# KikeM/romtime

Hardware: AMD Instinct MI355X
Metric: snapshot-DoF/s for POD build (higher is better)
Workload: dtype f64

## Files before the change

### include/romtime_hip.h

```cpp
#ifndef ROMTIME_HIP_H
#define ROMTIME_HIP_H

#include <stdint.h>

#ifdef __cplusplus
extern "C" {
#endif

typedef struct rt_ctx rt_ctx;

#define RT_OK 0
#define RT_ERR_ARG (-1)
#define RT_ERR_HIP (-2)
#define RT_ERR_UNSUPPORTED (-3)
#define RT_WARN_ZERO_NORM 1
#define RT_WARN_SINGULAR 2

#define RT_ROW_MAJOR 0
#define RT_COL_MAJOR 1

int rt_version(void);
int rt_ctx_create(rt_ctx** out, int device);
void rt_ctx_destroy(rt_ctx* ctx);
int rt_ctx_set_stream(rt_ctx* ctx, void* hip_stream);
int rt_ctx_synchronize(rt_ctx* ctx);
const char* rt_last_error(rt_ctx* ctx);
int rt_last_launch_info(rt_ctx* ctx, int64_t* info3);

int rt_ctx_set_profile(rt_ctx* ctx, int on);
int rt_ctx_set_option(rt_ctx* ctx, const char* name, int value);

int rt_stream_create_cu_range(int device, int first_cu_per_xcd, int n_cu_per_xcd, void** stream);
int rt_stream_destroy(void* stream);
int rt_last_gemm_ms(rt_ctx* ctx, double* ms);
int rt_ctx_get_counter(rt_ctx* ctx, const char* name, int64_t* value);
int rt_last_gram_ms(rt_ctx* ctx, double* ms);
int rt_gram_plan_info(int num_cus, int64_t n_rows, int64_t n_cols, int* out);


int rt_gram(rt_ctx* ctx, const double* X, int64_t n_rows, int64_t n_cols, int64_t ld, int layout,
            double* G);

int rt_gram_scale(rt_ctx* ctx, double* G, int64_t n, double* colnorm, int normalize, int* status_flag);

int rt_pod_orth(rt_ctx* ctx, const double* X, int64_t n_rows, int64_t n_cols, int64_t ld, int layout, int64_t num,
                double tol, int normalize, double* Q, int64_t q_cols, int64_t* r_out, double* s_host,
                double* energy_host, int* levels_out);

int rt_pod_enqueue(rt_ctx* ctx, const double* X, int64_t n_rows, int64_t n_cols, int64_t ld, int layout, int64_t k,
                   int normalize, double* G, double* colnorm, double* lam, int* status2, double* Z, double* Zs, double* Q);

int rt_pod_backproject_weights(rt_ctx* ctx, const double* Z, int64_t n, int64_t k, const double* colnorm, const double* lam,
                               double* Zs);

int rt_gemm_tn(rt_ctx* ctx, const double* A, int64_t lda, int a_layout, const double* B, int64_t ldb,
               int b_layout, int64_t N, int64_t m, int64_t n, double* C, int64_t ldc);

int rt_gemm_nn(rt_ctx* ctx, const double* X, int64_t ldx, int x_layout, const double* T, int64_t ldt,
               int64_t N, int64_t n, int64_t k, double* Y, int64_t ldy, int y_layout);
int rt_gemm_nn_axpby(rt_ctx* ctx, const double* X, int64_t ldx, int x_layout, const double* T, int64_t ldt,
                     int64_t N, int64_t n, int64_t k, double alpha, double beta, double* Y, int64_t ldy,
                     int y_layout);

int rt_rank_update(rt_ctx* ctx, const double* Ysrc, int64_t ldys, const double* colscale, const double* X, int64_t ldx,
                   const double* T, int64_t ldt, int64_t N, int64_t k, int64_t n, double alpha, double* Ydst,
                   int64_t ldyd);

int rt_transpose(rt_ctx* ctx, const double* src, int64_t rows, int64_t cols, int64_t ld_src, double* dst,
                 int64_t ld_dst);


int rt_deim_greedy(rt_ctx* ctx, const double* Phi, int64_t N, int64_t m, int64_t ld, int layout,
                   int64_t* idx, double* PT_U, double* margin);


int rt_csr_spmm(rt_ctx* ctx, const int64_t* indptr, const int64_t* indices, const double* data, int64_t N,
                const double* V, int64_t ldv, int64_t r, double* Y, int64_t ldy);

int rt_project_csr(rt_ctx* ctx, const int64_t* indptr, const int64_t* indices, const double* data, int64_t N,
                   const double* V, int64_t ldv, int64_t r, double* AN);

int rt_project_csr_batched(rt_ctx* ctx, const int64_t* indptr, const int64_t* indices,
                           const double* data_batch, int64_t ld_data, int data_layout, int64_t B, int64_t N,
                           const double* V, int64_t ldv, int64_t r, double* AN_batch);

int rt_project_stage_info(rt_ctx* ctx, const int64_t* indptr, const int64_t* indices, int64_t N, int64_t* records,
                          int* any_unwindowed);


int rt_dense_solve_batched(rt_ctx* ctx, double* K, double* rhs, int64_t r, int64_t B, int* info);
int rt_dense_solve_multi(rt_ctx* ctx, const double* K, int64_t r, const double* B, double* X, int64_t nrhs, int* info);


int rt_tracked_solve_batched(rt_ctx* ctx, const double* K, double* Xinv, double* rhs, int64_t r, int64_t B, int have_prev,
                             int* info);

#define RT_SOLVER_DIRECT 0
#define RT_SOLVER_GMRES 1
typedef struct {
  double rtol, atol;
  int64_t restart, maxiter;
} rt_gmres_opts;
int rt_gmres_batched(rt_ctx* ctx, const double* K, const double* b, double* x, int64_t r, int64_t B,
                     const rt_gmres_opts* opts, int64_t* info, int* iters);
int rt_ctx_set_reduced_solver(rt_ctx* ctx, int kind, const rt_gmres_opts* opts);

typedef struct {
  int64_t N, nnz, r, n_mu, nt;
  double dt;
  int bdf2;
  const int64_t* indptr;
  const int64_t* indices;
  const double* V;
  const double* mass_values;
  int64_t n_terms;
  const double* term_values;
  const double* term_coef;
  const double* tril_values;
  int64_t n_rhs;
  const double* rhs_terms;
// ... 97 lines not shown
```

### romtime_amd/_lib.py

```python
from __future__ import annotations

import ctypes as C
import os
import threading
import weakref

_HERE = os.path.dirname(os.path.abspath(__file__))
LIB_PATH = os.path.join(_HERE, "lib", "libromtime_hip.so")

ROW_MAJOR, COL_MAJOR = 0, 1
RT_OK = 0
WARN_ZERO_NORM, WARN_SINGULAR = 1, 2
EIG_BLOCKED_OK, EIG_BLOCKED_NOT_REDUCIBLE, EIG_BLOCKED_SOLVE_FAILED = 0, 1, 2

_p = C.c_void_p
_i64 = C.c_int64
_int = C.c_int

SOLVER_DIRECT, SOLVER_GMRES = 0, 1


class GmresOpts(C.Structure):

    _fields_ = [("rtol", C.c_double), ("atol", C.c_double), ("restart", _i64), ("maxiter", _i64)]


SIGNATURES = {
    "rt_version": (_int, []),
    "rt_ctx_create": (_int, [C.POINTER(_p), _int]),
    "rt_ctx_destroy": (None, [_p]),
    "rt_ctx_set_stream": (_int, [_p, _p]),
    "rt_ctx_synchronize": (_int, [_p]),
    "rt_last_error": (C.c_char_p, [_p]),
    "rt_last_launch_info": (_int, [_p, C.POINTER(_i64)]),
    "rt_ctx_set_profile": (_int, [_p, _int]),
    "rt_ctx_set_option": (_int, [_p, C.c_char_p, _int]),
    "rt_last_gemm_ms": (_int, [_p, C.POINTER(C.c_double)]),
    "rt_last_gram_ms": (_int, [_p, C.POINTER(C.c_double)]),
    "rt_gram_plan_info": (_int, [_int, _i64, _i64, C.POINTER(_int)]),
    "rt_ctx_get_counter": (_int, [_p, C.c_char_p, C.POINTER(_i64)]),
    "rt_stream_create_cu_range": (_int, [_int, _int, _int, C.POINTER(_p)]),
    "rt_stream_destroy": (_int, [_p]),
    "rt_last_sweep_stats": (_int, [_p, C.POINTER(_i64)]),
    "rt_gram": (_int, [_p, _p, _i64, _i64, _i64, _int, _p]),
    "rt_gram_scale": (_int, [_p, _p, _i64, _p, _int, _p]),
    "rt_pod_backproject_weights": (_int, [_p, _p, _i64, _i64, _p, _p, _p]),
    "rt_pod_enqueue": (_int, [_p, _p, _i64, _i64, _i64, _int, _i64, _int, _p, _p, _p, _p, _p, _p, _p]),
    "rt_pod_orth": (_int, [_p, _p, _i64, _i64, _i64, _int, _i64, C.c_double, _int, _p, _i64, C.POINTER(_i64), _p, _p,
                           C.POINTER(_int)]),
    "rt_gemm_tn": (_int, [_p, _p, _i64, _int, _p, _i64, _int, _i64, _i64, _i64, _p, _i64]),
    "rt_gemm_nn": (_int, [_p, _p, _i64, _int, _p, _i64, _i64, _i64, _i64, _p, _i64, _int]),
    "rt_rank_update": (_int, [_p, _p, _i64, _p, _p, _i64, _p, _i64, _i64, _i64, _i64, C.c_double, _p, _i64]),
    "rt_gemm_nn_axpby": (_int, [_p, _p, _i64, _int, _p, _i64, _i64, _i64, _i64, C.c_double, C.c_double, _p, _i64, _int]),
    "rt_transpose": (_int, [_p, _p, _i64, _i64, _i64, _p, _i64]),
    "rt_deim_greedy": (_int, [_p, _p, _i64, _i64, _i64, _int, _p, _p, _p]),
    "rt_csr_spmm": (_int, [_p, _p, _p, _p, _i64, _p, _i64, _i64, _p, _i64]),
    "rt_project_csr": (_int, [_p, _p, _p, _p, _i64, _p, _i64, _i64, _p]),
    "rt_project_csr_batched": (_int, [_p, _p, _p, _p, _i64, _int, _i64, _i64, _p, _i64, _i64, _p]),
    "rt_project_stage_info": (_int, [_p, _p, _p, _i64, C.POINTER(_i64), C.POINTER(_int)]),
    "rt_dense_solve_batched": (_int, [_p, _p, _p, _i64, _i64, _p]),
    "rt_dense_solve_multi": (_int, [_p, _p, _i64, _p, _p, _i64, _p]),
    "rt_tracked_solve_batched": (_int, [_p, _p, _p, _p, _i64, _i64, _int, _p]),
    "rt_gmres_batched": (_int, [_p, _p, _p, _p, _i64, _i64, C.POINTER(GmresOpts), _p, _p]),
    "rt_ctx_set_reduced_solver": (_int, [_p, _int, C.POINTER(GmresOpts)]),
    "rt_rom_bdf_sweep": (_int, [_p, _p, _p]),
    "rt_hrom_bdf_sweep": (_int, [_p, _p, _p]),
    "rt_trajectory_errors": (_int, [_p, _p, _i64, _p, _i64, _i64, _p, _i64, _int, _i64, _i64, _i64, _i64, _i64, _p, _p]),
    "rt_trajectory_integrals": (_int, [_p, _p, _i64, _p, _p, _i64, _i64, _p, _i64, _i64, _i64, _i64, _int, C.POINTER(C.c_double), _p]),
    "rt_trajectory_integrals_plan_info": (_int, [_int, _p, _i64, _p, _p, _i64, _i64, _p, _i64, _i64, _i64, _i64, _int,
                                                 C.POINTER(C.c_double), _p, C.POINTER(_i64)]),
    "rt_interpolation_errors": (_int, [_p, _p, _i64, C.POINTER(_i64), _i64, _p, _i64, _int, _i64, _i64, _i64, _i64, C.c_double, _p, _p]),
    "rt_interpolation_errors_plan_info": (_int, [_int, _p, _i64, C.POINTER(_i64), _i64, _p, _i64, _int, _i64, _i64, _i64, _i64,
                                                 C.c_double, _p, _p, C.POINTER(_i64)]),
    "rt_p1_local_assembly": (_int, [_p, _int, _i64, _p, _p, _i64, _i64, _p, _p, _int, _p, _p]),
    "rt_p1_fom_bdf_sweep": (_int, [_p, _p, _p, _i64, _i64, _p]),
    "rt_p1_fom_bdf_sweep_plan_info": (_int, [_int, _p, _i64, _i64, C.POINTER(_i64)]),
    "rt_p1_fom_bdf_sweep_certified": (_int, [_p, _p, _p, _i64, _i64, C.c_double, _p, _p]),
    "rt_p1_fom_bdf_sweep_certified_plan_info": (_int, [_int, _p, _i64, _i64, C.POINTER(_i64)]),
    "rt_trajectory_residuals": (_int, [_p, _p, _p, _i64, _i64, _p, _i64, _i64, _p, _p, _p]),
    "rt_trajectory_residuals_plan_info": (_int, [_int, _p, _p, _i64, _i64, _p, _i64, _i64, _p, _p, _p, C.POINTER(_i64)]),
    "rt_sym_eig_values": (_int, [_p, _p, _i64, _p, _p]),
    "rt_sym_eig_values_part": (_int, [_p, _p, _i64, _i64, _i64, _p, _p]),
    "rt_sym_eig_vectors": (_int, [_p, _i64, _i64, _p, _p]),
    "rt_sym_eig_blocked_plan_info": (_int, [_i64, _i64, C.POINTER(_i64), C.POINTER(_i64)]),
    "rt_sym_eig_blocked": (_int, [_p, _p, _i64, C.c_double, _i64, _p, _p, C.POINTER(_i64), C.POINTER(_i64), C.POINTER(_int)]),
    "rt_sym_jacobi_eigh": (_int, [_p, _p, _i64, _p, _p, _int, C.POINTER(_int), _p]),
    "rt_host_jacobi_eigh": (_int, [_p, _i64, _p, _p, _int, C.POINTER(_int)]),
    "rt_bench_mfma_f64": (_int, [_p, _int, C.POINTER(C.c_double)]),
    "rt_bench_copy": (_int, [_p, _p, _p, _i64, _int, C.POINTER(C.c_double)]),
}



class SweepDesc(C.Structure):

    _fields_ = [("N", _i64), ("nnz", _i64), ("r", _i64), ("n_mu", _i64), ("nt", _i64), ("dt", C.c_double),
                ("bdf2", _int), ("indptr", _p), ("indices", _p), ("V", _p), ("mass_values", _p), ("n_terms", _i64),
                ("term_values", _p), ("term_coef", _p), ("tril_values", _p), ("n_rhs", _i64), ("rhs_terms", _p),
                ("rhs_coef", _p)]


class HSweepDesc(C.Structure):

    _fields_ = [("r", _i64), ("n_mu", _i64), ("nt", _i64), ("dt", C.c_double), ("bdf2", _int), ("m_mass", _i64),
                ("m_lin", _i64), ("m_nl", _i64), ("m_rhs", _i64), ("Z", _p), ("Zf", _p), ("F_mass", _p), ("F_lin", _p),
                ("F_rhs", _p), ("W", _p), ("C_nl", _p), ("S_nl", _p)]


class FomDesc(C.Structure):

    _fields_ = [("nx", _i64), ("n_mu", _i64), ("nt", _i64), ("first_step", _i64), ("dt", C.c_double), ("bdf2", _int),
                ("state_in_w", _int), ("tab", _p), ("u_init", _p)]


_lib = None
_lock = threading.Lock()


class RomtimeHipError(RuntimeError):
    pass


# ... 157 lines not shown
```

### romtime_amd/csrc/api.hip

```cpp
#include "common.h"

#include <chrono>
#include <new>

namespace {

int grow(rt_ctx* ctx, void** buf, size_t* have, size_t bytes, void** out) {
  if (bytes > *have) {
    RT_HIP_CHECK(ctx, hipStreamSynchronize(ctx->stream));
    if (*buf) RT_HIP_CHECK(ctx, hipFree(*buf));
    *buf = nullptr;
    *have = 0;
    const size_t want = (bytes + ((size_t)1 << 20) - 1) & ~(((size_t)1 << 20) - 1);
    RT_HIP_CHECK(ctx, hipMalloc(buf, want));
    *have = want;
  }
  *out = *buf;
  return RT_OK;
}

__global__ void gram_scale_kernel(double* __restrict__ G, int n, double* __restrict__ colnorm, int normalize,
                                  int* status_flag) {
  const long idx = (long)blockIdx.x * blockDim.x + threadIdx.x;
  if (idx >= (long)n * n) return;
// ... 73 lines not shown
      for (int it = 0; it < iters; ++it) {
#pragma unroll
        for (int rep = 0; rep < 2; ++rep)
#pragma unroll
          for (int i = 0; i < 8; ++i) a[i] = fma(a[i], m, c);
      }
#pragma unroll
      for (int i = 0; i < 8; ++i) s += a[i];
    }
    if (mode & 4) {
      unsigned a[8];
#pragma unroll
      for (int i = 0; i < 8; ++i) a[i] = threadIdx.x * 2654435761u + i;
      for (int it = 0; it < iters; ++it) {
#pragma unroll
        for (int rep = 0; rep < 2; ++rep)
#pragma unroll
          for (int i = 0; i < 8; ++i) a[i] = (a[i] ^ (a[i] >> 3)) + 0x9e3779b9u;
      }
#pragma unroll
      for (int i = 0; i < 8; ++i) s += (double)a[i];
    }
    if (mode & 8) {
      int idx = threadIdx.x & 63;
      double a = 0.0;
      for (int it = 0; it < iters; ++it) {
#pragma unroll
        for (int i = 0; i < 16; ++i) a += lds[(idx + 64 * i) & 2047];
        idx = (idx + 1) & 63;
      }
      s += a;
    }
  }
  if (s == -1.2345) sink[0] = s;
}

__global__ __launch_bounds__(256) void copy_kernel(double4* __restrict__ dst, const double4* __restrict__ src, long n4) {
  const long stride = (long)gridDim.x * blockDim.x;
  for (long i = (long)blockIdx.x * blockDim.x + threadIdx.x; i < n4; i += stride) dst[i] = src[i];
}

}

int rt_scratch(rt_ctx* ctx, size_t bytes, void** out) { return grow(ctx, &ctx->scratch, &ctx->scratch_bytes, bytes, out); }
int rt_scratch2(rt_ctx* ctx, size_t bytes, void** out) {
  ++ctx->scratch2_gen;
  return grow(ctx, &ctx->scratch2, &ctx->scratch2_bytes, bytes, out);
}

int rt_func_lds(rt_ctx* ctx, const void* fn, int bytes) {
  for (const void* f : ctx->lds_done)
    if (f == fn) return RT_OK;
  RT_HIP_CHECK(ctx, hipFuncSetAttribute(fn, hipFuncAttributeMaxDynamicSharedMemorySize, bytes));
  ctx->lds_done.push_back(fn);
  return RT_OK;
}

int rt_profile_begin(rt_ctx* ctx, bool also_gram) {
  if (!ctx->profile) return RT_OK;
  if (!ctx->ev0) {
    RT_HIP_CHECK(ctx, hipEventCreate(&ctx->ev0));
    RT_HIP_CHECK(ctx, hipEventCreate(&ctx->ev1));
  }
  if (also_gram && !ctx->gev0) {
    RT_HIP_CHECK(ctx, hipEventCreate(&ctx->gev0));
    RT_HIP_CHECK(ctx, hipEventCreate(&ctx->gev1));
  }
  RT_HIP_CHECK(ctx, hipEventRecord(ctx->ev0, ctx->stream));
  if (also_gram) RT_HIP_CHECK(ctx, hipEventRecord(ctx->gev0, ctx->stream));
  return RT_OK;
}

int rt_profile_end(rt_ctx* ctx, bool also_gram) {
  if (!ctx->profile) return RT_OK;
  RT_HIP_CHECK(ctx, hipEventRecord(ctx->ev1, ctx->stream));
  if (also_gram) RT_HIP_CHECK(ctx, hipEventRecord(ctx->gev1, ctx->stream));
  ctx->ev_valid = true;
  if (also_gram) ctx->gev_valid = true;
  return RT_OK;
}

extern "C" {

int rt_version(void) { return 420; }

int rt_ctx_create(rt_ctx** out, int device) {
  if (!out) return RT_ERR_ARG;
  *out = nullptr;
  int count = 0;
  if (hipGetDeviceCount(&count) != hipSuccess || device < 0 || device >= count) return RT_ERR_HIP;
  if (hipSetDevice(device) != hipSuccess) return RT_ERR_HIP;
  rt_ctx* ctx = new (std::nothrow) rt_ctx();
  if (!ctx) return RT_ERR_HIP;
  ctx->device = device;
  hipDeviceProp_t prop;
  if (hipGetDeviceProperties(&prop, device) == hipSuccess) ctx->num_cus = ctx->device_cus = prop.multiProcessorCount;
  if (hipMalloc(reinterpret_cast<void**>(&ctx->dev_counters), sizeof(long) * RT_N_COUNTERS) != hipSuccess ||
      hipMemset(ctx->dev_counters, 0, sizeof(long) * RT_N_COUNTERS) != hipSuccess) {
    delete ctx;
    return RT_ERR_HIP;
  }
  *out = ctx;
  return RT_OK;
}

void rt_ctx_destroy(rt_ctx* ctx) {
  if (!ctx) return;
  (void)hipSetDevice(ctx->device);
  (void)hipDeviceSynchronize();
  if (ctx->scratch) (void)hipFree(ctx->scratch);
  if (ctx->scratch2) (void)hipFree(ctx->scratch2);
  if (ctx->dev_counters) (void)hipFree(ctx->dev_counters);
  if (ctx->gram_pace) (void)hipFree(ctx->gram_pace);
  if (ctx->ev0) (void)hipEventDestroy(ctx->ev0);
  if (ctx->ev1) (void)hipEventDestroy(ctx->ev1);
  if (ctx->gev0) (void)hipEventDestroy(ctx->gev0);
  if (ctx->gev1) (void)hipEventDestroy(ctx->gev1);
  delete ctx;
}

int rt_ctx_set_stream(rt_ctx* ctx, void* hip_stream) {
  if (!ctx) return RT_ERR_ARG;
  ctx->stream = static_cast<hipStream_t>(hip_stream);
  return RT_OK;
}

int rt_stream_create_cu_range(int device, int first_cu_per_xcd, int n_cu_per_xcd, void** stream) {
  if (!stream) return RT_ERR_ARG;
  *stream = nullptr;
  hipDeviceProp_t prop;
  if (hipSetDevice(device) != hipSuccess || hipGetDeviceProperties(&prop, device) != hipSuccess) return RT_ERR_HIP;
  const int per_xcd = prop.multiProcessorCount / 8;
  if (first_cu_per_xcd < 0 || n_cu_per_xcd < 1 || first_cu_per_xcd + n_cu_per_xcd > per_xcd) return RT_ERR_ARG;
  const int words = (prop.multiProcessorCount + 31) / 32;
  std::vector<uint32_t> mask((size_t)words, 0u);
  for (int cu = first_cu_per_xcd; cu < first_cu_per_xcd + n_cu_per_xcd; ++cu)
    for (int xcd = 0; xcd < 8; ++xcd) {
      const int bit = cu * 8 + xcd;
      mask[bit >> 5] |= 1u << (bit & 31);
    }
  hipStream_t st = nullptr;
  if (hipExtStreamCreateWithCUMask(&st, (uint32_t)words, mask.data()) != hipSuccess) return RT_ERR_HIP;
  *stream = st;
  return RT_OK;
}

int rt_stream_destroy(void* stream) {
  if (!stream) return RT_ERR_ARG;
  return hipStreamDestroy(static_cast<hipStream_t>(stream)) == hipSuccess ? RT_OK : RT_ERR_HIP;
}

int rt_ctx_synchronize(rt_ctx* ctx) {
  if (!ctx) return RT_ERR_ARG;
  RT_HIP_CHECK(ctx, hipStreamSynchronize(ctx->stream));
  return RT_OK;
}

const char* rt_last_error(rt_ctx* ctx) { return ctx ? ctx->err.c_str() : "null ctx"; }

int rt_last_launch_info(rt_ctx* ctx, int64_t* info3) {
  if (!ctx || !info3) return RT_ERR_ARG;
  info3[0] = ctx->last_grid;
  info3[1] = ctx->last_splits;
  info3[2] = ctx->last_tile;
  return RT_OK;
}

// ... 247 lines not shown
```

### romtime_amd/csrc/gram_mfma.hip

```cpp
#include <algorithm>
#include <type_traits>

#include "gemm_panel.h"

using namespace rtk;

namespace {

constexpr int BT = 128;
constexpr int GT = 512;
constexpr int MAX_SLOTS = 64;
constexpr int MAX_TILES = 36;
typedef unsigned u2 __attribute__((ext_vector_type(2)));
constexpr unsigned long long PACE_ONE = 1ull << 40;
constexpr int PACE_DROP = 6;

struct GramParams {
  const double* X;
  long ks, ms;
  long K, n, kx;
  long last0;
  double* slab;
  int nslots, tiles1, vec;
  long* counters;
  unsigned long long* pace;
  int pace_every, pace_slack, pace_naps;
  unsigned char slot_tm[MAX_SLOTS], slot_tn[MAX_SLOTS], slot_q[MAX_SLOTS], slot_S[MAX_SLOTS];
};

struct GramSegs {
  unsigned char tm[MAX_SLOTS], tn[MAX_SLOTS], q[MAX_SLOTS], S[MAX_SLOTS];
  unsigned short slab[MAX_SLOTS];
};

__device__ const unsigned char kDiagTi[8][5] = {{0, 0, 0, 0, 0}, {0, 0, 0, 1, 1}, {1, 1, 1, 1, 1}, {2, 2, 2, 2, 2}, {2, 3, 3, 3, 255}, {3, 3, 4, 4, 255}, {4, 4, 5, 5, 255}, {5, 6, 6, 7, 255}};
__device__ const unsigned char kDiagTj[8][5] = {{0, 1, 2, 3, 4}, {5, 6, 7, 1, 2}, {3, 4, 5, 6, 7}, {2, 3, 4, 5, 6}, {7, 3, 4, 5, 0}, {6, 7, 4, 5, 0}, {6, 7, 5, 6, 0}, {7, 6, 7, 7, 0}};

template <bool KC, bool DIAG>
__device__ __forceinline__ void gram_segment(const GramParams& p, double* smem, int x, int tm, int tn, int q0, int S,
                                             double* out) {
  using P = Panel<BT, KC, GT>;
  double* sA0 = smem;
  double* sA1 = smem + P::LDS;
  double* sB0 = smem + 2 * P::LDS;
  double* sB1 = smem + 3 * P::LDS;

  int tid = threadIdx.x;
  asm volatile("" : "+v"(tid));
  const long m0 = (tm == p.tiles1 - 1) ? p.last0 : (long)tm * BT, n0 = (tn == p.tiles1 - 1) ? p.last0 : (long)tn * BT;
  const long kend_x = ((long)x * p.kx + p.kx < p.K) ? (long)x * p.kx + p.kx : p.K;
  const int nst_x = (kend_x > (long)x * p.kx) ? (int)((kend_x - (long)x * p.kx + KB - 1) / KB) : 0;
  const long kbeg = (long)x * p.kx;
  const long kend = kend_x;
  const int nstages = (nst_x > q0) ? (nst_x - q0 + S - 1) / S : 0;

  const int lane = tid & 63, wid = tid >> 6;
  const int wm = wid >> 2, wn = wid & 3;
  const int l15 = lane & 15, l4 = lane >> 4;

  unsigned long long* pace = p.pace ? p.pace + 16 * x : nullptr;
  int pacer = (pace && __builtin_amdgcn_readfirstlane(wid) == 0 && nstages > 0) ? 1 : 0;
  int pace_pos = 0, pace_cnt = 0;
  if (pacer && lane == 0) __hip_atomic_fetch_add(pace, PACE_ONE, __ATOMIC_RELAXED, __HIP_MEMORY_SCOPE_AGENT);

  constexpr int NACC = DIAG ? 5 : 8;
  d4 acc[NACC];
#pragma unroll
  for (int i = 0; i < NACC; ++i) acc[i] = d4{0.0, 0.0, 0.0, 0.0};
  int dti[5], dtj[5];
  bool dval[5];
  {
    const int w = __builtin_amdgcn_readfirstlane(wid);
#pragma unroll
    for (int q = 0; q < 5; ++q) {
      dval[q] = kDiagTi[w][q] != 255;
      dti[q] = dval[q] ? 16 * kDiagTi[w][q] : 0;
      dtj[q] = 16 * kDiagTj[w][q];
    }
  }

  d2 ra[P::NL], rb[DIAG ? 1 : P::NL];
  const bool interior = p.vec && (m0 + BT <= p.n) && (n0 + BT <= p.n);
  if (nstages > 0) {
    const long k0 = kbeg + (long)q0 * KB;
    P::load(ra, p.X, p.ks, p.ms, k0, kend, m0, p.n, p.vec, tid);
    if constexpr (!DIAG) P::load(rb, p.X, p.ks, p.ms, k0, kend, n0, p.n, p.vec, tid);
    P::store(ra, sA0, tid);
    if constexpr (!DIAG) P::store(rb, sB0, tid);
  }
  __syncthreads();

  const long k1 = kbeg + (long)(q0 + S) * KB;
  const char* gA = reinterpret_cast<const char*>(p.X + k1 * p.ks + m0 * p.ms);
  const char* gB = reinterpret_cast<const char*>(p.X + k1 * p.ks + n0 * p.ms);
  const unsigned voff = P::lane_offset(p.ks, p.ms, tid);
  const long rows_step = P::load_step(p.ks, p.ms), stage_step = (long)S * KB * p.ks * 8;

  int n_full = nstages;
  if (nstages > 0 && kbeg + (long)(q0 + (nstages - 1) * S) * KB + KB > kend) n_full = nstages - 1;
  if (!interior) n_full = 0;

  auto compute = [&](const double* cA, const double* cB) {
    if constexpr (DIAG) {
#pragma unroll
      for (int k4 = 0; k4 < KB / 4; ++k4) {
#pragma unroll
        for (int q = 0; q < 5; ++q) {
          if (!dval[q]) continue;
          const double a = P::frag(cA, dti[q], k4, l15, l4);
          const double b = P::frag(cA, dtj[q], k4, l15, l4);
          acc[q] = __builtin_amdgcn_mfma_f64_16x16x4f64(a, b, acc[q], 0, 0, 0);
        }
      }
    } else {
#pragma unroll
      for (int k4 = 0; k4 < KB / 4; ++k4) {
        double a[4], b[2];
#pragma unroll
        for (int i = 0; i < 4; ++i) a[i] = P::frag(cA, wm * 64 + i * 16, k4, l15, l4);
#pragma unroll
        for (int j = 0; j < 2; ++j) b[j] = P::frag(cB, wn * 32 + j * 16, k4, l15, l4);
#pragma unroll
        for (int i = 0; i < 4; ++i)
#pragma unroll
          for (int j = 0; j < 2; ++j)
            acc[i * 2 + j] = __builtin_amdgcn_mfma_f64_16x16x4f64(a[i], b[j], acc[i * 2 + j], 0, 0, 0);
      }
    }
  };

  int st = 0;
  {
    auto fast_stage = [&](auto parity) {
      constexpr int PAR = decltype(parity)::value;
      P::load_full_u(ra, gA, voff, rows_step);
      if constexpr (!DIAG) P::load_full_u(rb, gB, voff, rows_step);
      const bool check = pacer && ++pace_cnt == p.pace_every;
      unsigned long long before = 0;
      if (check) {
        pace_cnt = 0;
        const int adv = S * p.pace_every;
        if (lane == 0) before = __hip_atomic_fetch_add(pace, (unsigned long long)adv, __ATOMIC_RELAXED, __HIP_MEMORY_SCOPE_AGENT);
        pace_pos += adv;
      }
      __builtin_amdgcn_s_setprio(1);
      compute(PAR ? sA1 : sA0, PAR ? sB1 : sB0);
      __builtin_amdgcn_s_setprio(0);
      gA += stage_step;
      gB += stage_step;
      P::store(ra, PAR ? sA0 : sA1, tid);
      if constexpr (!DIAG) P::store(rb, PAR ? sB0 : sB1, tid);
      if (check) {
        unsigned lo = __builtin_amdgcn_readfirstlane((unsigned)before), hi = __builtin_amdgcn_readfirstlane((unsigned)(before >> 32));
        unsigned long long word = (((unsigned long long)hi << 32) | lo) + (unsigned long long)(S * p.pace_every);
#pragma unroll 1
        for (int nap = 0;; ++nap) {
          const long long total = (long long)(word & (PACE_ONE - 1)), members = (long long)(word >> 40);
          const long long lead = (long long)pace_pos * members - total;
          if (lead < -(long long)PACE_DROP * S * members) {
            if (lane == 0)
              __hip_atomic_fetch_add(pace, 0ull - (PACE_ONE + (unsigned long long)pace_pos), __ATOMIC_RELAXED,
                                     __HIP_MEMORY_SCOPE_AGENT);
            pacer = 0;
            break;
          }
          if (lead <= (long long)p.pace_slack * S * members || nap >= p.pace_naps) break;
          __builtin_amdgcn_s_sleep(16);
          u2 v;
          asm volatile("s_load_dwordx2 %0, %1, 0x0 glc\n\ts_waitcnt lgkmcnt(0)" : "=s"(v) : "s"(pace) : "memory");
          word = ((unsigned long long)v.y << 32) | v.x;
        }
      }
      __syncthreads();
    };
    for (; st + 2 < n_full; st += 2) {
      fast_stage(std::integral_constant<int, 0>{});
      fast_stage(std::integral_constant<int, 1>{});
    }
  }
  for (; st < nstages; ++st) {
    const double* cA = (st & 1) ? sA1 : sA0;
    const double* cB = (st & 1) ? sB1 : sB0;
    const bool more = st + 1 < nstages;
    if (more) {
      const long k0 = kbeg + (long)(q0 + (st + 1) * S) * KB;
      if (st + 1 < n_full) {
        P::load_full(ra, p.X, p.ks, p.ms, k0, m0, tid);
        if constexpr (!DIAG) P::load_full(rb, p.X, p.ks, p.ms, k0, n0, tid);
      } else {
        P::load(ra, p.X, p.ks, p.ms, k0, kend, m0, p.n, p.vec, tid);
        if constexpr (!DIAG) P::load(rb, p.X, p.ks, p.ms, k0, kend, n0, p.n, p.vec, tid);
      }
    }
    __builtin_amdgcn_s_setprio(1);
    compute(cA, cB);
    __builtin_amdgcn_s_setprio(0);
    if (more) {
      P::store(ra, (st & 1) ? sA0 : sA1, tid);
      if constexpr (!DIAG) P::store(rb, (st & 1) ? sB0 : sB1, tid);
    }
    __syncthreads();
  }

  if constexpr (DIAG) {
#pragma unroll
    for (int q = 0; q < 5; ++q)
#pragma unroll
      for (int r = 0; r < 4; ++r)
        if (dval[q]) out[(dti[q] + l4 + 4 * r) * BT + dtj[q] + l15] = acc[q][r];
  } else {
#pragma unroll
    for (int i = 0; i < 4; ++i)
#pragma unroll
      for (int j = 0; j < 2; ++j)
#pragma unroll
        for (int r = 0; r < 4; ++r)
          out[(wm * 64 + i * 16 + l4 + 4 * r) * BT + wn * 32 + j * 16 + l15] = acc[i * 2 + j][r];
  }
}

__device__ __forceinline__ void gram_check_xcd(const GramParams& p, int x) {
  if (threadIdx.x == 0 && (int)(__builtin_amdgcn_s_getreg((31 << 11) | 20) & 15u) != x)
    atomicAdd(reinterpret_cast<unsigned long long*>(&p.counters[RT_CNT_GRAM_OFF_XCD]), 1ull);
}

template <bool KC, bool DIAG>
__global__ __launch_bounds__(GT, 4) void gram128_kernel(const GramParams p) {
  extern __shared__ __attribute__((aligned(16))) double smem[];
  const int x = blockIdx.x & 7, slot = blockIdx.x >> 3;
  gram_check_xcd(p, x);
  const int tm = __builtin_amdgcn_readfirstlane((int)p.slot_tm[slot]), tn = __builtin_amdgcn_readfirstlane((int)p.slot_tn[slot]),
            q0 = __builtin_amdgcn_readfirstlane((int)p.slot_q[slot]), S = __builtin_amdgcn_readfirstlane((int)p.slot_S[slot]);
  gram_segment<KC, DIAG>(p, smem, x, tm, tn, q0, S, p.slab + ((long)x * p.nslots + slot) * (BT * BT));
}

template <bool KC>
__global__ __launch_bounds__(GT, 4) void gram128_merged_kernel(const GramParams p, const GramSegs g) {
  extern __shared__ __attribute__((aligned(16))) double smem[];
  const int x = blockIdx.x & 7, slot = blockIdx.x >> 3;
  gram_check_xcd(p, x);
  const int S = __builtin_amdgcn_readfirstlane((int)g.S[slot]);
  if (S == 0) return;
  const int tm = __builtin_amdgcn_readfirstlane((int)g.tm[slot]), tn = __builtin_amdgcn_readfirstlane((int)g.tn[slot]),
            q0 = __builtin_amdgcn_readfirstlane((int)g.q[slot]), slab = __builtin_amdgcn_readfirstlane((int)g.slab[slot]);
  double* out = p.slab + ((long)x * p.nslots + slab) * (BT * BT);
  if (tm == tn)
    gram_segment<KC, true>(p, smem, x, tm, tn, q0, S, out);
  else
    gram_segment<KC, false>(p, smem, x, tm, tn, q0, S, out);
}

struct GramReduceParams {
  const double* slab_off;
  const double* slab_diag;
  double* G;
  long n, last0;
  int nslots_off, nslots_diag, tiles1;
  unsigned char first[MAX_TILES], count[MAX_TILES];
  unsigned long long* pace;
};

__global__ void gram_reduce_kernel(const GramReduceParams p) {
  const long idx = (long)blockIdx.x * blockDim.x + threadIdx.x;
  if (p.pace && idx < 256) p.pace[idx] = 0ull;
  if (idx >= p.n * p.n) return;
  const long i = idx / p.n, j = idx % p.n;
  if (i > j) return;
  const int tm = (int)(i / BT), tn = (int)(j / BT);
  const int t = tm * p.tiles1 - tm * (tm - 1) / 2 + (tn - tm);
  const long off = (i - (tm == p.tiles1 - 1 ? p.last0 : (long)tm * BT)) * BT + (j - (tn == p.tiles1 - 1 ? p.last0 : (long)tn * BT));
  const double* slab = (tm == tn) ? p.slab_diag : p.slab_off;
  const int nslots = (tm == tn) ? p.nslots_diag : p.nslots_off;
  const int cnt = p.count[t];
  const double* base = slab + (long)p.first[t] * (BT * BT) + off;
  double sum = 0.0;
  for (int x = 0; x < 8; ++x) {
    const double* src = base + (long)x * nslots * (BT * BT);
#pragma unroll 4
    for (int q = 0; q < cnt; ++q) sum += src[(long)q * (BT * BT)];
  }
  p.G[idx] = sum;
  if (i != j) p.G[j * p.n + i] = sum;
}

template <bool KC, bool DIAG>
int launch_gram(rt_ctx* ctx, const GramParams& p, int grid) {
  const size_t lds = sizeof(double) * (DIAG ? 2 : 4) * Panel<BT, KC, GT>::LDS;
  RT_TRY(rt_func_lds(ctx, reinterpret_cast<const void*>(&gram128_kernel<KC, DIAG>), (int)lds));
  hipLaunchKernelGGL((gram128_kernel<KC, DIAG>), dim3(grid), dim3(GT), lds, ctx->stream, p);
  RT_HIP_CHECK(ctx, hipGetLastError());
  return RT_OK;
}

constexpr double GRAM_RHO = 0.60;

struct GramPace {
  int every, slack, naps;
};
constexpr GramPace PACE_TWO_LAUNCHES{2, 2, 8}, PACE_ONE_LAUNCH{2, 1, 8};

double gram_uniform_ab(int P, int n_off, int n_d, double rho, int cap, int* a_out, int* b_out) {
  double best = 1e30;
  int best_slots = 0;
  *a_out = *b_out = 0;
  for (int a = 1; a <= cap && n_off * a + n_d <= P; ++a)
    for (int b = 1; b <= cap && n_off * a + n_d * b <= P; ++b) {
      const double T = (1.0 / a > rho / b) ? 1.0 / a : rho / b;
      const int used = n_off * a + n_d * b;
      if (T < best - 1e-12 || (T < best + 1e-12 && used < best_slots)) { best = T; *a_out = a; *b_out = b; best_slots = used; }
    }
  return *a_out ? best : 0.0;
}

int gram_plan(int tiles1, int s_off, int s_diag, GramSegs& g, unsigned char* first, unsigned char* count) {
  g = GramSegs{};
  int slot = 0;
  for (int diag = 0; diag < 2; ++diag) {
    const int S = diag ? s_diag : s_off;
    int t = 0;
    for (int a = 0; a < tiles1; ++a)
      for (int b = a; b < tiles1; ++b, ++t) {
        if ((a == b) != (diag == 1)) continue;
        first[t] = (unsigned char)slot;
        count[t] = (unsigned char)S;
        for (int q = 0; q < S; ++q, ++slot) {
          g.tm[slot] = (unsigned char)a; g.tn[slot] = (unsigned char)b;
          g.q[slot] = (unsigned char)q; g.S[slot] = (unsigned char)S;
          g.slab[slot] = (unsigned short)slot;
        }
      }
  }
  return slot;
}

struct GramChoice {
  int form, a, b, s_off, s_diag, slots;
};
GramChoice gram_choose(int num_cus, long K, long n) {
  const int slots_max = 2 * num_cus / 8;
  GramChoice c{0, 0, 0, 0, 0, slots_max};
  const int tiles1 = (int)((n + BT - 1) / BT), ntiles = tiles1 * (tiles1 + 1) / 2, n_off = ntiles - tiles1;
  if (n < 97 || ntiles > MAX_TILES || n_off > slots_max || slots_max > MAX_SLOTS || K < 8L * 64 * KB) return c;
  const long kx = ((K + 7) / 8 + KB - 1) / KB * KB;
  const int cap = (int)(kx / KB / 48);
  if (cap < 1) return c;
  c.s_off = n_off ? std::min(slots_max / n_off, cap) : 0;
  c.s_diag = std::min(slots_max / tiles1, cap);
  if (n_off >= 1) {
    const double t_uni = gram_uniform_ab(slots_max, n_off, tiles1, GRAM_RHO, cap, &c.a, &c.b);
    const double t_two = (c.s_off >= 1 && c.s_diag >= 1) ? 1.0 / c.s_off + GRAM_RHO / c.s_diag : 0.0;
    if (t_uni > 0.0 && t_two > 0.0 && t_uni <= 1.05 * t_two && n_off * c.a + tiles1 * c.b >= 16 && !(tiles1 == 2 && c.a >= cap)) {
      c.form = 2;
      return c;
    }
  }
  const int busiest = n_off ? n_off * c.s_off : tiles1 * c.s_diag;
  c.form = (busiest >= 16) ? 1 : 0;
  return c;
}

template <bool KC>
int launch_gram_merged(rt_ctx* ctx, const GramParams& p, const GramSegs& g, int grid) {
  constexpr size_t lds = sizeof(double) * 4 * Panel<BT, KC, GT>::LDS;
  RT_TRY(rt_func_lds(ctx, reinterpret_cast<const void*>(&gram128_merged_kernel<KC>), (int)lds));
  hipLaunchKernelGGL((gram128_merged_kernel<KC>), dim3(grid), dim3(GT), lds, ctx->stream, p, g);
  RT_HIP_CHECK(ctx, hipGetLastError());
  return RT_OK;
}

}

int rt_gram128(rt_ctx* ctx, const double* X, int64_t ks, int64_t ms, int64_t K, int64_t n, double* G) {
  if (!(ks == 1 || ms == 1)) return RT_ERR_UNSUPPORTED;
  const GramChoice c = gram_choose(ctx->num_cus, (long)K, (long)n);
  if (c.form == 0) return RT_ERR_UNSUPPORTED;
  const bool one_launch = c.form == 2;
  const bool kc = (ks == 1) && (ms != 1);
  const int tiles1 = (int)((n + BT - 1) / BT), n_off = tiles1 * (tiles1 - 1) / 2;

  GramParams p;
  p.X = X; p.ks = ks; p.ms = ms; p.K = K; p.n = n;
  p.kx = ((K + 7) / 8 + KB - 1) / KB * KB;
  p.tiles1 = tiles1;
  const long other = kc ? ms : ks;
  p.vec = ((((uintptr_t)X) & 15) == 0 && (other % 2 == 0)) ? 1 : 0;
  p.last0 = (long)(tiles1 - 1) * BT;
  if (n % BT != 0 && n >= BT && p.vec && (kc || n % 2 == 0)) p.last0 = n - BT;
  if ((!kc && (long)ks * 8 * 8 >= (1L << 31)) || (kc && (long)ms * 64 * 8 >= (1L << 31))) p.vec = 0;
  p.counters = ctx->dev_counters;
  p.pace = nullptr;
  const GramPace pace = one_launch ? PACE_ONE_LAUNCH : PACE_TWO_LAUNCHES;
  p.pace_every = pace.every; p.pace_slack = pace.slack; p.pace_naps = pace.naps;
  if (ctx->gram_pace_on) {
    if (!ctx->gram_pace) {
      RT_HIP_CHECK(ctx, hipMalloc(reinterpret_cast<void**>(&ctx->gram_pace), sizeof(unsigned long long) * 256));
      RT_HIP_CHECK(ctx, hipMemsetAsync(ctx->gram_pace, 0, sizeof(unsigned long long) * 256, ctx->stream));
    }
    p.pace = ctx->gram_pace;
  }

  GramSegs g;
  GramReduceParams rp;
  int nslots_off, nslots_diag;
  if (one_launch) {
    nslots_off = nslots_diag = gram_plan(tiles1, c.a, c.b, g, rp.first, rp.count);
  } else {
    nslots_off = c.s_off * n_off;
    nslots_diag = c.s_diag * tiles1;
  }
  void* slab = nullptr;
  int rc = rt_scratch(ctx, sizeof(double) * BT * BT * 8 * (size_t)(one_launch ? nslots_off : nslots_off + nslots_diag), &slab);
  if (rc != RT_OK) return rc;
  double* slab_off = static_cast<double*>(slab);
  double* slab_diag = one_launch ? slab_off : slab_off + (size_t)8 * nslots_off * BT * BT;
  rp.slab_off = slab_off; rp.slab_diag = slab_diag; rp.G = G; rp.n = n; rp.last0 = p.last0;
  rp.nslots_off = nslots_off; rp.nslots_diag = nslots_diag; rp.tiles1 = tiles1; rp.pace = ctx->gram_pace;

  RT_TRY(rt_profile_begin(ctx, true));
  if (one_launch) {
    p.slab = slab_off; p.nslots = nslots_off;
    rc = kc ? launch_gram_merged<true>(ctx, p, g, 8 * c.slots) : launch_gram_merged<false>(ctx, p, g, 8 * c.slots);
    if (rc != RT_OK) return rc;
  } else {
    if (n_off) {
      int slot = 0, t = 0;
      for (int a = 0; a < tiles1; ++a)
        for (int b = a; b < tiles1; ++b, ++t) {
          if (a == b) continue;
          rp.first[t] = (unsigned char)slot; rp.count[t] = (unsigned char)c.s_off;
          for (int q = 0; q < c.s_off; ++q, ++slot) {
            p.slot_tm[slot] = (unsigned char)a; p.slot_tn[slot] = (unsigned char)b;
            p.slot_q[slot] = (unsigned char)q; p.slot_S[slot] = (unsigned char)c.s_off;
          }
        }
      p.slab = slab_off; p.nslots = nslots_off;
      rc = kc ? launch_gram<true, false>(ctx, p, 8 * nslots_off) : launch_gram<false, false>(ctx, p, 8 * nslots_off);
      if (rc != RT_OK) return rc;
    }
    {
      int slot = 0, t = 0;
      for (int a = 0; a < tiles1; ++a)
        for (int b = a; b < tiles1; ++b, ++t) {
          if (a != b) continue;
          rp.first[t] = (unsigned char)slot; rp.count[t] = (unsigned char)c.s_diag;
          for (int q = 0; q < c.s_diag; ++q, ++slot) {
            p.slot_tm[slot] = (unsigned char)a; p.slot_tn[slot] = (unsigned char)a;
            p.slot_q[slot] = (unsigned char)q; p.slot_S[slot] = (unsigned char)c.s_diag;
          }
        }
      p.slab = slab_diag; p.nslots = nslots_diag;
      p.pace = nullptr;
      rc = kc ? launch_gram<true, true>(ctx, p, 8 * nslots_diag) : launch_gram<false, true>(ctx, p, 8 * nslots_diag);
      if (rc != RT_OK) return rc;
    }
  }
  RT_TRY(rt_profile_end(ctx, true));
  ctx->last_grid = one_launch ? 8 * c.slots : 8 * (nslots_off + nslots_diag);
  ctx->last_splits = 8 * (one_launch ? c.a : c.s_off);
  ctx->last_tile = 128 * 1000 + 128;
  const long total = n * n;
  hipLaunchKernelGGL(gram_reduce_kernel, dim3((unsigned)((total + 255) / 256)), dim3(256), 0, ctx->stream, rp);
  RT_HIP_CHECK(ctx, hipGetLastError());
  return RT_OK;
}

extern "C" int rt_gram_plan_info(int num_cus, int64_t n_rows, int64_t n_cols, int* out) {
  if (!out || num_cus < 8 || n_rows < 1 || n_cols < 1) return RT_ERR_ARG;
  const GramChoice c = gram_choose(num_cus, (long)n_rows, (long)n_cols);
  out[0] = c.form; out[1] = c.a; out[2] = c.b; out[3] = c.s_off; out[4] = c.s_diag;
  return RT_OK;
}
```

Before: 91.37 billion.

## Add spare workgroups that finish tile K-tails to balance two-launch Gram

In the two-launch Gram path, the number of regular K-split slots per tile no longer fills all available slots, so leftover slots are now used as spare workgroups. Each regular slot processes a shortened main K range, and each spare workgroup loops over several tiles to compute their remaining K-tail stages into an extra slab that the reduce step sums. The aim is to fill idle CUs and cut the tail imbalance at the end of each launch. The diagonal kernel also raises its launch-bounds occupancy hint. This adds extra slab traffic and a serial loop inside the spare workgroups, and the split heuristic may not suit every shape.

```diff
diff --git a/include/romtime_hip.h b/include/romtime_hip.h
--- a/include/romtime_hip.h
+++ b/include/romtime_hip.h
@@ -36,6 +36,7 @@
 int rt_ctx_get_counter(rt_ctx* ctx, const char* name, int64_t* value);
 int rt_last_gram_ms(rt_ctx* ctx, double* ms);
 int rt_gram_plan_info(int num_cus, int64_t n_rows, int64_t n_cols, int* out);
+int rt_gram_spare_plan_info(int num_cus, int64_t n_rows, int64_t n_cols, int launch, int xcd, int* out);
 
 
 int rt_gram(rt_ctx* ctx, const double* X, int64_t n_rows, int64_t n_cols, int64_t ld, int layout,
diff --git a/romtime_amd/_lib.py b/romtime_amd/_lib.py
--- a/romtime_amd/_lib.py
+++ b/romtime_amd/_lib.py
@@ -38,6 +38,7 @@
     "rt_last_gemm_ms": (_int, [_p, C.POINTER(C.c_double)]),
     "rt_last_gram_ms": (_int, [_p, C.POINTER(C.c_double)]),
     "rt_gram_plan_info": (_int, [_int, _i64, _i64, C.POINTER(_int)]),
+    "rt_gram_spare_plan_info": (_int, [_int, _i64, _i64, _int, _int, C.POINTER(_int)]),
     "rt_ctx_get_counter": (_int, [_p, C.c_char_p, C.POINTER(_i64)]),
     "rt_stream_create_cu_range": (_int, [_int, _int, _int, C.POINTER(_p)]),
     "rt_stream_destroy": (_int, [_p]),
diff --git a/romtime_amd/csrc/api.hip b/romtime_amd/csrc/api.hip
--- a/romtime_amd/csrc/api.hip
+++ b/romtime_amd/csrc/api.hip
@@ -179,7 +179,7 @@
 
 extern "C" {
 
-int rt_version(void) { return 420; }
+int rt_version(void) { return 430; }
 
 int rt_ctx_create(rt_ctx** out, int device) {
   if (!out) return RT_ERR_ARG;
diff --git a/romtime_amd/csrc/gram_mfma.hip b/romtime_amd/csrc/gram_mfma.hip
--- a/romtime_amd/csrc/gram_mfma.hip
+++ b/romtime_amd/csrc/gram_mfma.hip
@@ -25,7 +25,9 @@
   long* counters;
   unsigned long long* pace;
   int pace_every, pace_slack, pace_naps;
-  unsigned char slot_tm[MAX_SLOTS], slot_tn[MAX_SLOTS], slot_q[MAX_SLOTS], slot_S[MAX_SLOTS];
+  int n_regular;
+  int n_main[8];
+  unsigned char slot_tm[MAX_SLOTS], slot_tn[MAX_SLOTS], slot_q[MAX_SLOTS], slot_S[MAX_SLOTS], slot_slab[MAX_SLOTS];
 };
 
 struct GramSegs {
@@ -36,29 +38,30 @@
 __device__ const unsigned char kDiagTi[8][5] = {{0, 0, 0, 0, 0}, {0, 0, 0, 1, 1}, {1, 1, 1, 1, 1}, {2, 2, 2, 2, 2}, {2, 3, 3, 3, 255}, {3, 3, 4, 4, 255}, {4, 4, 5, 5, 255}, {5, 6, 6, 7, 255}};
 __device__ const unsigned char kDiagTj[8][5] = {{0, 1, 2, 3, 4}, {5, 6, 7, 1, 2}, {3, 4, 5, 6, 7}, {2, 3, 4, 5, 6}, {7, 3, 4, 5, 0}, {6, 7, 4, 5, 0}, {6, 7, 5, 6, 0}, {7, 6, 7, 7, 0}};
 
+__device__ __forceinline__ int gram_range_stages(const GramParams& p, int x) {
+  const long kbeg = (long)x * p.kx, kend = (kbeg + p.kx < p.K) ? kbeg + p.kx : p.K;
+  return (kend > kbeg) ? (int)((kend - kbeg + KB - 1) / KB) : 0;
+}
+
 template <bool KC, bool DIAG>
 __device__ __forceinline__ void gram_segment(const GramParams& p, double* smem, int x, int tm, int tn, int q0, int S,
-                                             double* out) {
+                                             int nstages, bool paced, int tid, double* out) {
   using P = Panel<BT, KC, GT>;
   double* sA0 = smem;
   double* sA1 = smem + P::LDS;
   double* sB0 = smem + 2 * P::LDS;
   double* sB1 = smem + 3 * P::LDS;
 
-  int tid = threadIdx.x;
   asm volatile("" : "+v"(tid));
   const long m0 = (tm == p.tiles1 - 1) ? p.last0 : (long)tm * BT, n0 = (tn == p.tiles1 - 1) ? p.last0 : (long)tn * BT;
-  const long kend_x = ((long)x * p.kx + p.kx < p.K) ? (long)x * p.kx + p.kx : p.K;
-  const int nst_x = (kend_x > (long)x * p.kx) ? (int)((kend_x - (long)x * p.kx + KB - 1) / KB) : 0;
   const long kbeg = (long)x * p.kx;
-  const long kend = kend_x;
-  const int nstages = (nst_x > q0) ? (nst_x - q0 + S - 1) / S : 0;
+  const long kend = (kbeg + p.kx < p.K) ? kbeg + p.kx : p.K;
 
   const int lane = tid & 63, wid = tid >> 6;
   const int wm = wid >> 2, wn = wid & 3;
   const int l15 = lane & 15, l4 = lane >> 4;
 
-  unsigned long long* pace = p.pace ? p.pace + 16 * x : nullptr;
+  unsigned long long* pace = (p.pace && paced) ? p.pace + 16 * x : nullptr;
   int pacer = (pace && __builtin_amdgcn_readfirstlane(wid) == 0 && nstages > 0) ? 1 : 0;
   int pace_pos = 0, pace_cnt = 0;
   if (pacer && lane == 0) __hip_atomic_fetch_add(pace, PACE_ONE, __ATOMIC_RELAXED, __HIP_MEMORY_SCOPE_AGENT);
@@ -225,13 +228,36 @@
 }
 
 template <bool KC, bool DIAG>
-__global__ __launch_bounds__(GT, 4) void gram128_kernel(const GramParams p) {
+__global__ __launch_bounds__(GT, (DIAG && !KC) ? 6 : 4) void gram128_kernel(const GramParams p) {
   extern __shared__ __attribute__((aligned(16))) double smem[];
   const int x = blockIdx.x & 7, slot = blockIdx.x >> 3;
   gram_check_xcd(p, x);
-  const int tm = __builtin_amdgcn_readfirstlane((int)p.slot_tm[slot]), tn = __builtin_amdgcn_readfirstlane((int)p.slot_tn[slot]),
-            q0 = __builtin_amdgcn_readfirstlane((int)p.slot_q[slot]), S = __builtin_amdgcn_readfirstlane((int)p.slot_S[slot]);
-  gram_segment<KC, DIAG>(p, smem, x, tm, tn, q0, S, p.slab + ((long)x * p.nslots + slot) * (BT * BT));
+  const int S = __builtin_amdgcn_readfirstlane((int)p.slot_S[slot]);
+  const int n_main = p.n_main[x];
+  const int wave = __builtin_amdgcn_readfirstlane(threadIdx.x >> 6);
+  if (slot < p.n_regular) {
+    const int lane = __builtin_amdgcn_mbcnt_hi(~0u, __builtin_amdgcn_mbcnt_lo(~0u, 0u));
+    const int tm = __builtin_amdgcn_readfirstlane((int)p.slot_tm[slot]), tn = __builtin_amdgcn_readfirstlane((int)p.slot_tn[slot]),
+              q0 = __builtin_amdgcn_readfirstlane((int)p.slot_q[slot]), slab = __builtin_amdgcn_readfirstlane((int)p.slot_slab[slot]);
+    const int nstages = (n_main > q0) ? (n_main - q0 + S - 1) / S : 0;
+    gram_segment<KC, DIAG>(p, smem, x, tm, tn, q0, S, nstages, true, wave * 64 + lane, p.slab + ((long)x * p.nslots + slab) * (BT * BT));
+    return;
+  }
+#pragma unroll 1
+  for (int i = 0;; ++i) {
+    int wg = blockIdx.x, zero = 0;
+    asm volatile("" : "+s"(wg), "+s"(zero));
+    const int tid = wave * 64 + __builtin_amdgcn_mbcnt_hi(~0u, __builtin_amdgcn_mbcnt_lo(~0u, zero));
+    const int xs = wg & 7, ss = wg >> 3;
+    const int Ss = __builtin_amdgcn_readfirstlane((int)p.slot_S[ss]);
+    if (i >= __builtin_amdgcn_readfirstlane((int)p.slot_tn[ss])) break;
+    const int r = (__builtin_amdgcn_readfirstlane((int)p.slot_tm[ss]) + i) * Ss;
+    const int tm = __builtin_amdgcn_readfirstlane((int)p.slot_tm[r]), tn = __builtin_amdgcn_readfirstlane((int)p.slot_tn[r]),
+              slab = __builtin_amdgcn_readfirstlane((int)p.slot_slab[r + Ss - 1]) + 1;
+    const int first = p.n_main[xs];
+    gram_segment<KC, DIAG>(p, smem, xs, tm, tn, first, 1, gram_range_stages(p, xs) - first, false, tid,
+                           p.slab + ((long)xs * p.nslots + slab) * (BT * BT));
+  }
 }
 
 template <bool KC>
@@ -244,10 +270,12 @@
   const int tm = __builtin_amdgcn_readfirstlane((int)g.tm[slot]), tn = __builtin_amdgcn_readfirstlane((int)g.tn[slot]),
             q0 = __builtin_amdgcn_readfirstlane((int)g.q[slot]), slab = __builtin_amdgcn_readfirstlane((int)g.slab[slot]);
   double* out = p.slab + ((long)x * p.nslots + slab) * (BT * BT);
+  const int nst_x = gram_range_stages(p, x);
+  const int nstages = (nst_x > q0) ? (nst_x - q0 + S - 1) / S : 0;
   if (tm == tn)
-    gram_segment<KC, true>(p, smem, x, tm, tn, q0, S, out);
+    gram_segment<KC, true>(p, smem, x, tm, tn, q0, S, nstages, true, threadIdx.x, out);
   else
-    gram_segment<KC, false>(p, smem, x, tm, tn, q0, S, out);
+    gram_segment<KC, false>(p, smem, x, tm, tn, q0, S, nstages, true, threadIdx.x, out);
 }
 
 struct GramReduceParams {
@@ -359,6 +387,56 @@
   return c;
 }
 
+int gram_n_main(int nst, int m, int s) {
+  const long ms = (long)m * s;
+  return (int)((2 * nst * ms + 1 + ms) / (2 * (1 + ms)));
+}
+struct GramSpare {
+  int spare, m;
+};
+GramSpare gram_spare_plan(int slots_max, int n_t, int s, int cap, long kx) {
+  GramSpare sp{0, 0};
+  if (n_t < 1 || s < 1 || slots_max / n_t > cap) return sp;
+  const int R = std::min(slots_max - n_t * s, n_t);
+  if (R < 1) return sp;
+  const int m = (n_t + R - 1) / R;
+  const int nst = (int)(kx / KB);
+  if ((long)(n_t / R) * (nst - gram_n_main(nst, m, s)) < 48) return sp;
+  sp.spare = R; sp.m = m;
+  return sp;
+}
+
+int gram_fill_launch(GramParams& p, int tiles1, bool diag, int s, const GramSpare& sp, unsigned char* first,
+                     unsigned char* count, int* nslabs) {
+  const int per_tile = s + (sp.spare ? 1 : 0);
+  int slot = 0, n_t = 0, t = 0;
+  for (int a = 0; a < tiles1; ++a)
+    for (int b = a; b < tiles1; ++b, ++t) {
+      if ((a == b) != diag) continue;
+      first[t] = (unsigned char)(n_t * per_tile); count[t] = (unsigned char)per_tile;
+      for (int q = 0; q < s; ++q, ++slot) {
+        p.slot_tm[slot] = (unsigned char)a; p.slot_tn[slot] = (unsigned char)b;
+        p.slot_q[slot] = (unsigned char)q; p.slot_S[slot] = (unsigned char)s;
+        p.slot_slab[slot] = (unsigned char)(n_t * per_tile + q);
+      }
+      ++n_t;
+    }
+  p.n_regular = slot;
+  for (int x = 0; x < 8; ++x) {
+    const long kbeg = (long)x * p.kx, kend = std::min(kbeg + p.kx, p.K);
+    const int nst_x = (kend > kbeg) ? (int)((kend - kbeg + KB - 1) / KB) : 0;
+    p.n_main[x] = sp.spare ? gram_n_main(nst_x, sp.m, s) : nst_x;
+  }
+  for (int j = 0, t0 = 0; j < sp.spare; ++j, ++slot) {
+    const int cnt = n_t / sp.spare + (j < n_t % sp.spare ? 1 : 0);
+    p.slot_tm[slot] = (unsigned char)t0; p.slot_tn[slot] = (unsigned char)cnt;
+    p.slot_q[slot] = 0; p.slot_S[slot] = (unsigned char)s; p.slot_slab[slot] = 0;
+    t0 += cnt;
+  }
+  *nslabs = n_t * per_tile;
+  return slot;
+}
+
 template <bool KC>
 int launch_gram_merged(rt_ctx* ctx, const GramParams& p, const GramSegs& g, int grid) {
   constexpr size_t lds = sizeof(double) * 4 * Panel<BT, KC, GT>::LDS;
@@ -402,11 +480,15 @@
   GramSegs g;
   GramReduceParams rp;
   int nslots_off, nslots_diag;
+  int wgs_off = 0, wgs_diag = 0;
+  GramParams p_diag = p;
   if (one_launch) {
     nslots_off = nslots_diag = gram_plan(tiles1, c.a, c.b, g, rp.first, rp.count);
   } else {
-    nslots_off = c.s_off * n_off;
-    nslots_diag = c.s_diag * tiles1;
+    const int cap = (int)(p.kx / KB / 48);
+    nslots_off = 0;
+    if (n_off) wgs_off = gram_fill_launch(p, tiles1, false, c.s_off, gram_spare_plan(c.slots, n_off, c.s_off, cap, p.kx), rp.first, rp.count, &nslots_off);
+    wgs_diag = gram_fill_launch(p_diag, tiles1, true, c.s_diag, gram_spare_plan(c.slots, tiles1, c.s_diag, cap, p.kx), rp.first, rp.count, &nslots_diag);
   }
   void* slab = nullptr;
   int rc = rt_scratch(ctx, sizeof(double) * BT * BT * 8 * (size_t)(one_launch ? nslots_off : nslots_off + nslots_diag), &slab);
@@ -423,39 +505,17 @@
     if (rc != RT_OK) return rc;
   } else {
     if (n_off) {
-      int slot = 0, t = 0;
-      for (int a = 0; a < tiles1; ++a)
-        for (int b = a; b < tiles1; ++b, ++t) {
-          if (a == b) continue;
-          rp.first[t] = (unsigned char)slot; rp.count[t] = (unsigned char)c.s_off;
-          for (int q = 0; q < c.s_off; ++q, ++slot) {
-            p.slot_tm[slot] = (unsigned char)a; p.slot_tn[slot] = (unsigned char)b;
-            p.slot_q[slot] = (unsigned char)q; p.slot_S[slot] = (unsigned char)c.s_off;
-          }
-        }
       p.slab = slab_off; p.nslots = nslots_off;
-      rc = kc ? launch_gram<true, false>(ctx, p, 8 * nslots_off) : launch_gram<false, false>(ctx, p, 8 * nslots_off);
+      rc = kc ? launch_gram<true, false>(ctx, p, 8 * wgs_off) : launch_gram<false, false>(ctx, p, 8 * wgs_off);
       if (rc != RT_OK) return rc;
     }
-    {
-      int slot = 0, t = 0;
-      for (int a = 0; a < tiles1; ++a)
-        for (int b = a; b < tiles1; ++b, ++t) {
-          if (a != b) continue;
-          rp.first[t] = (unsigned char)slot; rp.count[t] = (unsigned char)c.s_diag;
-          for (int q = 0; q < c.s_diag; ++q, ++slot) {
-            p.slot_tm[slot] = (unsigned char)a; p.slot_tn[slot] = (unsigned char)a;
-            p.slot_q[slot] = (unsigned char)q; p.slot_S[slot] = (unsigned char)c.s_diag;
-          }
-        }
-      p.slab = slab_diag; p.nslots = nslots_diag;
-      p.pace = nullptr;
-      rc = kc ? launch_gram<true, true>(ctx, p, 8 * nslots_diag) : launch_gram<false, true>(ctx, p, 8 * nslots_diag);
-      if (rc != RT_OK) return rc;
-    }
+    p_diag.slab = slab_diag; p_diag.nslots = nslots_diag;
+    p_diag.pace = nullptr;
+    rc = kc ? launch_gram<true, true>(ctx, p_diag, 8 * wgs_diag) : launch_gram<false, true>(ctx, p_diag, 8 * wgs_diag);
+    if (rc != RT_OK) return rc;
   }
   RT_TRY(rt_profile_end(ctx, true));
-  ctx->last_grid = one_launch ? 8 * c.slots : 8 * (nslots_off + nslots_diag);
+  ctx->last_grid = one_launch ? 8 * c.slots : 8 * (wgs_off + wgs_diag);
   ctx->last_splits = 8 * (one_launch ? c.a : c.s_off);
   ctx->last_tile = 128 * 1000 + 128;
   const long total = n * n;
@@ -470,3 +530,22 @@
   out[0] = c.form; out[1] = c.a; out[2] = c.b; out[3] = c.s_off; out[4] = c.s_diag;
   return RT_OK;
 }
+
+extern "C" int rt_gram_spare_plan_info(int num_cus, int64_t n_rows, int64_t n_cols, int launch, int xcd, int* out) {
+  if (!out || num_cus < 8 || n_rows < 1 || n_cols < 1 || launch < 0 || launch > 1 || xcd < 0 || xcd > 7) return RT_ERR_ARG;
+  const GramChoice c = gram_choose(num_cus, (long)n_rows, (long)n_cols);
+  const int tiles1 = (int)((n_cols + BT - 1) / BT), n_t = launch ? tiles1 : tiles1 * (tiles1 - 1) / 2;
+  if (c.form != 1 || n_t < 1) return RT_ERR_UNSUPPORTED;
+  GramParams p;
+  p.K = (long)n_rows;
+  p.kx = ((p.K + 7) / 8 + KB - 1) / KB * KB;
+  const int s = launch ? c.s_diag : c.s_off;
+  const GramSpare sp = gram_spare_plan(c.slots, n_t, s, (int)(p.kx / KB / 48), p.kx);
+  unsigned char first[MAX_TILES], count[MAX_TILES];
+  int nslabs;
+  gram_fill_launch(p, tiles1, launch == 1, s, sp, first, count, &nslabs);
+  const long kbeg = (long)xcd * p.kx, kend = std::min(kbeg + p.kx, p.K);
+  out[0] = n_t; out[1] = s; out[2] = sp.spare; out[3] = sp.m; out[4] = p.n_main[xcd];
+  out[5] = (kend > kbeg) ? (int)((kend - kbeg + KB - 1) / KB) : 0;
+  return RT_OK;
+}
```

After: 93.56 billion, median of 6. 1.02x the previous value.
